# atenpas/gpd

Hardware: AMD Instinct MI355X
Metric: 15-ch grasp candidates scored/sec (imagegen+LeNet) at 1/2/4/8 MI355X (higher is better)
Workload: dtype f64 geometry / u8 images / LeNet f32-equivalent by exact operand splitting: conv1 int8 digit planes of 32-bit fixed-point weights (i32 accumulate, exact), conv2 + ip1 three bf16 pieces per operand (six exact products per term, f32 accumulate), ip2 f32

## Files before the change

### gpd_amd/csrc/images.hip

```cpp
#include <cfloat>
#include <cmath>
#include <cstdio>
#include <cstdlib>
#include <cstring>

#include <mutex>
#include <type_traits>

#include "gpd_internal.h"

namespace gpd {

#define HIP_RET(expr)                                                                       \
  do {                                                                                      \
    hipError_t e_ = (expr);                                                                 \
    if (e_ != hipSuccess) {                                                                 \
      set_error("%s failed: %s (%s:%d)", #expr, hipGetErrorString(e_), __FILE__, __LINE__); \
      return GPD_ERR_HIP;                                                                   \
    }                                                                                       \
  } while (0)

constexpr int IMG_THREADS = 512;
constexpr int SET_THREADS = 1024;
constexpr int IMG_WAVES = IMG_THREADS / 64;
constexpr int PT_CAP = 1024;
constexpr int PT_CAP_BIG = 32768;
constexpr int SH_CAP = 6144;
constexpr int SH_CAP_BIG = 12288;
template <bool WIDE>
struct Vox {
  static constexpr int VD = WIDE ? 64 : 46;
  static constexpr int SD = WIDE ? 128 : 86;
  static constexpr int SR = WIDE ? 64 : 43;
  static constexpr int LB = 18;
  static constexpr int SETWORDS = (SD * SD * SD + 31) / 32;
};

struct ImgConsts {
  double vol_depth, vol_width, vol_height, half_od, dbl_h;
  int C, nproj, per;
  double shadow_length, voxel, voxel_mult, rand_inv;
  int num_shadow;
  uint32_t stride_a, stride_c;
  double len[3];
  double inv_cell[3];
  double thr[3][kImg + 1];
  double inv_len[3];
  int true_div;
  int set_sd, set_sr;
};
__constant__ ImgConsts c_img;

struct ImgParams {
  const float *nn;
  int cap;
  const double *centers;
  const gpd_hand *hands;
  const int32_t *cand_hand;
  const int32_t *meta;
  const uint32_t *set_bits;
  uint8_t *images;
  int32_t *status;
  int num_cand;
  const int32_t *cand_list;
  const int32_t *cand_count;
  int32_t *overflow_list;
  int32_t *overflow_count;
  unsigned long long *dbg;
  int32_t *pts_overflow_list;
  int32_t *pts_overflow_count;
  char *pts_scratch;
  int exit_after;
  char *huge_scratch;
};

struct Box {
  double F[9];
  double sample[3];
  double off[3];
  double lo[3], hi[3];
};

constexpr size_t PTS_SCRATCH_BYTES = (size_t)PT_CAP_BIG * (3 * sizeof(double) + sizeof(float4) + sizeof(uint32_t));
struct PointArrays {
  double t[3][PT_CAP];
  float4 an[PT_CAP];
};
struct NoPointArrays {};
template <bool BIG>
struct __attribute__((aligned(16))) SmemPts {
  typename std::conditional<BIG, NoPointArrays, PointArrays>::type p;
  __attribute__((aligned(16))) uint32_t cells[kPix];
  uint16_t place[BIG ? PT_CAP_BIG : PT_CAP];
  float4 nzv[(BIG ? kPix : PT_CAP) + 1];
  uint16_t nzlist[BIG ? kPix : PT_CAP];
  double thr[3][kImg + 1];
  double recip[128];
  float red_f[4 * IMG_WAVES];
  int red_i[IMG_WAVES];
  int counter;
  int flag;
};
typedef SmemPts<false> Smem;
template <int SHC, bool WIDE>
struct __attribute__((aligned(16))) SmemShadow {
  __attribute__((aligned(16))) float raster0[kPix];
  __attribute__((aligned(16))) uint32_t cells[kPix];
  uint32_t lin[SHC];
  union {
    struct {
      uint16_t rowbase[Vox<WIDE>::VD * Vox<WIDE>::VD];
      uint8_t rowcnt[Vox<WIDE>::VD * Vox<WIDE>::VD];
    } rows;
    uint16_t place[SHC];
  } bp;
  uint16_t nz[kPix];
  uint8_t cz[SHC];
  double thr[3][kImg + 1];
  double recip[128];
  float red_f[4 * IMG_WAVES];
  int red_i[IMG_WAVES];
  int vorg[3];
  int flag;
};

__device__ inline double uniform_f64(double v) {
  const unsigned long long b = (unsigned long long)__double_as_longlong(v);
  const unsigned lo = __builtin_amdgcn_readfirstlane((unsigned)b);
  const unsigned hi = __builtin_amdgcn_readfirstlane((unsigned)(b >> 32));
  return __longlong_as_double((long long)(((unsigned long long)hi << 32) | lo));
}

template <class OP>
__device__ inline float wave_reduce_f32(float v, OP op) {
  auto dpp = [](float x, auto ctrl, auto rmask) {
    return __int_as_float(__builtin_amdgcn_update_dpp(__float_as_int(x), __float_as_int(x), decltype(ctrl)::value, decltype(rmask)::value, 0xf, false));
  };
  using std::integral_constant;
  v = op(v, dpp(v, integral_constant<int, 0xB1>(), integral_constant<int, 0xf>()));
  v = op(v, dpp(v, integral_constant<int, 0x4E>(), integral_constant<int, 0xf>()));
  v = op(v, dpp(v, integral_constant<int, 0x141>(), integral_constant<int, 0xf>()));
  v = op(v, dpp(v, integral_constant<int, 0x140>(), integral_constant<int, 0xf>()));
  v = op(v, dpp(v, integral_constant<int, 0x142>(), integral_constant<int, 0xa>()));
  v = op(v, dpp(v, integral_constant<int, 0x143>(), integral_constant<int, 0xc>()));
  return __int_as_float(__builtin_amdgcn_readlane(__float_as_int(v), 63));
}
__device__ inline float wave_max_f32(float v) { return wave_reduce_f32(v, [](float a, float b) { return fmaxf(a, b); }); }
__device__ inline float wave_min_f32(float v) { return wave_reduce_f32(v, [](float a, float b) { return fminf(a, b); }); }

__device__ inline int wave_incl_scan_i32(int v) {
  v += __builtin_amdgcn_update_dpp(0, v, 0x111, 0xf, 0xf, false);
  v += __builtin_amdgcn_update_dpp(0, v, 0x112, 0xf, 0xf, false);
  v += __builtin_amdgcn_update_dpp(0, v, 0x114, 0xf, 0xf, false);
  v += __builtin_amdgcn_update_dpp(0, v, 0x118, 0xf, 0xf, false);
  v += __builtin_amdgcn_update_dpp(0, v, 0x142, 0xa, 0xf, false);
  v += __builtin_amdgcn_update_dpp(0, v, 0x143, 0xc, 0xf, false);
  return v;
}

__device__ inline void to_hand(const Box &B, double w0, double w1, double w2, double t[3]) {
  const double c0 = w0 - B.sample[0], c1 = w1 - B.sample[1], c2 = w2 - B.sample[2];
  t[0] = B.F[0] * c0 + B.F[3] * c1 + B.F[6] * c2;
  t[1] = B.F[1] * c0 + B.F[4] * c1 + B.F[7] * c2;
  t[2] = B.F[2] * c0 + B.F[5] * c1 + B.F[8] * c2;
}
__device__ inline bool in_box(const Box &B, const double t[3]) {
  return (t[0] > B.lo[0]) && (t[0] < B.hi[0]) && (t[1] > B.lo[1]) && (t[1] < B.hi[1]) && (t[2] > B.lo[2]) && (t[2] < B.hi[2]);
}
template <class SM>
__device__ inline int cell_coord(const SM &S, int axis, double x) {
  int k = (int)(x * c_img.inv_cell[axis]);
  k = k < 0 ? 0 : (k > kImg - 1 ? kImg - 1 : k);
  const double t0 = S.thr[axis][k], t1 = S.thr[axis][k + 1];
  if (k > 0 && x < t0) {
    k--;
    while (k > 0 && x < S.thr[axis][k]) k--;
  } else if (k < kImg - 1 && x >= t1) {
    k++;
    while (k < kImg - 1 && x >= S.thr[axis][k + 1]) k++;
  }
  return k;
}
template <class SM>
__device__ inline uint32_t cells_of(const SM &S, const Box &B, const double t[3]) {
  const int cx = cell_coord(S, 0, t[0] - B.off[0]);
  const int cy = cell_coord(S, 1, t[1] - B.off[1]);
  const int cz = cell_coord(S, 2, t[2] - B.off[2]);
  return (uint32_t)cx | ((uint32_t)cy << 6) | ((uint32_t)cz << 12);
}
__device__ inline int cell_of_key(uint32_t key, int pr) {
  const int cx = key & 63, cy = (key >> 6) & 63, cz = (key >> 12) & 63;
  const int v = pr == 0 ? cx : cz;
  const int h = pr == 2 ? cx : cy;
  return h + v * kImg;
}
__device__ inline int depth_axis(int pr) { return pr == 0 ? 2 : (pr == 1 ? 0 : 1); }

__device__ inline double div_len(double x, int axis) {
  const ImgConsts &K = c_img;
  if (K.true_div) return x / K.len[axis];
  const double y = K.inv_len[axis];
  const double q = x * y;
  const double r = __builtin_fma(-K.len[axis], q, x);
  return __builtin_fma(r, y, q);
}
template <int NTAB>
__device__ inline double recip_count(const double *tab, float fc) {
  const int k = (int)fc;
  return k < NTAB ? tab[k] : 1.0 / (double)fc;
}

__device__ inline uint32_t lcg_step(uint32_t &s) {
  s = 214013u * s + 2531011u;
  return (uint32_t)(((int32_t)s >> 16) & 0x7FFF);
}
__device__ inline uint32_t lcg_jump(uint32_t s, unsigned long long n) {
  uint32_t a = 214013u, c = 2531011u, A = 1u, Cc = 0u;
  while (n) {
    if (n & 1ull) {
      A = a * A;
      Cc = a * Cc + c;
    }
    c = (a + 1u) * c;
    a = a * a;
    n >>= 1;
  }
  return A * s + Cc;
}

template <class SM>
__device__ inline int block_excl_scan(SM &S, int v, int *total) {
  const int lane = threadIdx.x & 63, wave = threadIdx.x >> 6;
  const int incl = wave_incl_scan_i32(v);
  __syncthreads();
  if (lane == 63) S.red_i[wave] = incl;
  __syncthreads();
  int base = 0, tot = 0;
#pragma unroll
  for (int w = 0; w < IMG_WAVES; w++) {
    const int x = S.red_i[w];
    if (w < wave) base += x;
    tot += x;
  }
  *total = tot;
  return base + incl - v;
}

template <class SM>
__device__ int scan_cells(SM &S) {
  const int tid = threadIdx.x;
  constexpr int PER = 8;
  static_assert(kPix % PER == 0 && kPix / PER <= IMG_THREADS, "scan_cells: cells per thread");
  uint4 *c4 = reinterpret_cast<uint4 *>(S.cells);
  if (tid < 32) reinterpret_cast<int *>(S.red_f)[tid] = 0;
  uint4 a = make_uint4(0u, 0u, 0u, 0u), b = a;
  if (tid < kPix / PER) {
    a = c4[2 * tid];
    b = c4[2 * tid + 1];
  }
  const int c[PER] = {(int)(a.x & 0xffffu), (int)(a.y & 0xffffu), (int)(a.z & 0xffffu), (int)(a.w & 0xffffu),
                      (int)(b.x & 0xffffu), (int)(b.y & 0xffffu), (int)(b.z & 0xffffu), (int)(b.w & 0xffffu)};
  int sum = 0;
#pragma unroll
  for (int k = 0; k < PER; k++) sum += c[k];
  int total;
  int run = block_excl_scan(S, sum, &total);
  uint32_t o[PER];
#pragma unroll
  for (int k = 0; k < PER; k++) {
    o[k] = (uint32_t)(run < 0xffff ? run : 0xffff) << 16;
    run += c[k];
  }
  if (tid < kPix / PER) {
    c4[2 * tid] = make_uint4(o[0], o[1], o[2], o[3]);
    c4[2 * tid + 1] = make_uint4(o[4], o[5], o[6], o[7]);
  }
  __syncthreads();
  return total;
}

template <class SM>
__device__ int list_nonempty_cells(SM &S, uint16_t *nz) {
  const int tid = threadIdx.x;
  constexpr int PER = (kPix + IMG_THREADS - 1) / IMG_THREADS;
  int *hist = reinterpret_cast<int *>(S.red_f);
  static_assert(PER == 8, "two 16-byte reads per thread");
  uint4 a = make_uint4(0u, 0u, 0u, 0u), b = a;
  if (tid < kPix / PER) {
    a = reinterpret_cast<const uint4 *>(S.cells)[2 * tid];
    b = reinterpret_cast<const uint4 *>(S.cells)[2 * tid + 1];
  }
  const uint32_t cw[PER] = {a.x, a.y, a.z, a.w, b.x, b.y, b.z, b.w};
  int bucket[PER];
#pragma unroll
  for (int k = 0; k < PER; k++) {
    const int cn = (int)(cw[k] & 0xffffu);
    bucket[k] = cn ? 31 - (cn < 31 ? cn : 31) : -1;
    if (cn) atomicAdd(&hist[bucket[k]], 1);
  }
  __syncthreads();
  if (tid < 64) {
    const int v = tid < 32 ? hist[tid] : 0;
    const int incl = wave_incl_scan_i32(v);
    if (tid < 32) hist[tid] = incl - v;
    if (tid == 31) S.red_i[0] = incl;
  }
  __syncthreads();
#pragma unroll
  for (int k = 0; k < PER; k++)
    if (bucket[k] >= 0) nz[atomicAdd(&hist[bucket[k]], 1)] = (uint16_t)(tid * PER + k);
  __syncthreads();
  return S.red_i[0];
}

template <int NPL, class SM>
__device__ void finalize_planes(SM &S, const float *p012, const float *p3, uint8_t *out) {
  const int tid = threadIdx.x;
  constexpr int GROUPS = NPL * 900;
  constexpr int PER = (GROUPS + IMG_THREADS - 1) / IMG_THREADS;
  float d[PER][4];
  float mn[2] = {FLT_MAX, FLT_MAX}, mx[2] = {-FLT_MAX, -FLT_MAX};
#pragma unroll
  for (int k = 0; k < PER; k++) {
    const int g = tid + k * IMG_THREADS;
    if (g < GROUPS) {
      const int ch = g / 900, rem = g - ch * 900;
      const int r = rem / 15, c0 = (rem - r * 15) * 4;
      const float *pl = (ch < 3) ? p012 + ch * kPix : p3;
      const int rm = r > 0 ? r - 1 : 0, rp = r < kImg - 1 ? r + 1 : kImg - 1;
      const int cl = c0 > 0 ? c0 - 1 : 0, cr = c0 + 4 < kImg ? c0 + 4 : kImg - 1;
      const float4 a = *reinterpret_cast<const float4 *>(pl + rm * kImg + c0);
      const float4 b = *reinterpret_cast<const float4 *>(pl + r * kImg + c0);
      const float4 c = *reinterpret_cast<const float4 *>(pl + rp * kImg + c0);
      const float el = fmaxf(fmaxf(pl[rm * kImg + cl], pl[r * kImg + cl]), pl[rp * kImg + cl]);
      const float er = fmaxf(fmaxf(pl[rm * kImg + cr], pl[r * kImg + cr]), pl[rp * kImg + cr]);
      const float m0 = fmaxf(fmaxf(a.x, b.x), c.x), m1 = fmaxf(fmaxf(a.y, b.y), c.y);
      const float m2 = fmaxf(fmaxf(a.z, b.z), c.z), m3 = fmaxf(fmaxf(a.w, b.w), c.w);
      d[k][0] = fmaxf(fmaxf(el, m0), m1);
      d[k][1] = fmaxf(fmaxf(m0, m1), m2);
      d[k][2] = fmaxf(fmaxf(m1, m2), m3);
      d[k][3] = fmaxf(fmaxf(m2, m3), er);
      const float lo = fminf(fminf(d[k][0], d[k][1]), fminf(d[k][2], d[k][3]));
      const float hi = fmaxf(fmaxf(d[k][0], d[k][1]), fmaxf(d[k][2], d[k][3]));
      if (ch < 3) {
        mn[0] = fminf(mn[0], lo);
        mx[0] = fmaxf(mx[0], hi);
      } else {
        mn[1] = fminf(mn[1], lo);
        mx[1] = fmaxf(mx[1], hi);
      }
    }
  }
#pragma unroll
  for (int q = 0; q < 2; q++) {
    mn[q] = wave_min_f32(mn[q]);
    mx[q] = wave_max_f32(mx[q]);
  }
  __syncthreads();
  if ((tid & 63) == 0) {
    S.red_f[4 * (tid >> 6) + 0] = mn[0];
    S.red_f[4 * (tid >> 6) + 1] = mx[0];
    S.red_f[4 * (tid >> 6) + 2] = mn[1];
    S.red_f[4 * (tid >> 6) + 3] = mx[1];
  }
  __syncthreads();
  float fs[2], fb[2];
#pragma unroll
  for (int q = 0; q < 2; q++) {
    float a = S.red_f[2 * q], b = S.red_f[2 * q + 1];
#pragma unroll
    for (int w = 1; w < IMG_WAVES; w++) {
      a = fminf(a, S.red_f[4 * w + 2 * q]);
      b = fmaxf(b, S.red_f[4 * w + 2 * q + 1]);
    }
    const double smin = (double)a, smax = (double)b;
    const double scale = 1.0 * ((smax - smin) > DBL_EPSILON ? 1.0 / (smax - smin) : 0.0);
    const double shift = 0.0 - smin * scale;
    fs[q] = (float)scale;
    fb[q] = (float)shift;
  }
#pragma unroll
  for (int k = 0; k < PER; k++) {
    const int g = tid + k * IMG_THREADS;
// ... 152 lines not shown
  for (int q = 0; q < 16; q++) k[q] = 16 + q < n ? (uint32_t)p[16 + q] : 0xffffffffu;
  merge_regs<16>(k);
#pragma unroll
  for (int q = 0; q < 16; q++)
    if (16 + q < n) p[16 + q] = (uint16_t)k[q];
}
template <int N>
__device__ inline void sort_regs(uint32_t (&k)[N]) {
#pragma unroll
  for (int size = 2; size <= N; size <<= 1) {
#pragma unroll
    for (int stride = size >> 1; stride > 0; stride >>= 1) {
#pragma unroll
      for (int i = 0; i < N; i++) {
        const int j = i ^ stride;
        if (j > i) {
          const uint32_t lo = min(k[i], k[j]), hi = max(k[i], k[j]);
          const bool up = (i & size) == 0;
          k[i] = up ? lo : hi;
          k[j] = up ? hi : lo;
        }
      }
    }
  }
}
template <int N>
__device__ inline void sort_u16_regs(uint16_t *p, int n) {
  uint32_t k[N];
#pragma unroll
  for (int q = 0; q < N; q++) k[q] = q < n ? (uint32_t)p[q] : 0xffffffffu;
  sort_regs<N>(k);
#pragma unroll
  for (int q = 0; q < N; q++)
    if (q < n) p[q] = (uint16_t)k[q];
}
#define TICK(k)                                                     \
  do {                                                              \
    if (P.dbg && tid == 0) {                                        \
      const unsigned long long now_ = __builtin_readcyclecounter(); \
      atomicAdd(&P.dbg[k], now_ - t_last);                          \
      t_last = now_;                                                \
    }                                                               \
  } while (0)

__device__ inline void load_box(const gpd_hand &H, Box &B) {
  const ImgConsts &K = c_img;
#pragma unroll
  for (int i = 0; i < 9; i++) B.F[i] = uniform_f64(H.frame[i]);
#pragma unroll
  for (int i = 0; i < 3; i++) B.sample[i] = uniform_f64(H.sample[i]);
  const double hb = uniform_f64(H.bottom), hc = uniform_f64(H.center);
  B.off[0] = hb;
  B.off[1] = uniform_f64(hc - K.half_od);
  B.off[2] = uniform_f64(-K.vol_height);
  B.lo[0] = hb;
  B.hi[0] = uniform_f64(hb + K.vol_depth);
  B.lo[1] = B.off[1];
  B.hi[1] = uniform_f64(hc + K.half_od);
  B.lo[2] = uniform_f64(-1.0 * K.vol_height);
  B.hi[2] = uniform_f64(K.vol_height);
}

__device__ __forceinline__ int xcd_candidate(int n) {
  const int per = (n + 7) >> 3;
  const int L = blockIdx.x, slot = L >> 3;
  const int cand = (L & 7) * per + slot;
  return cand < n ? cand : -1;
}

template <int SHC, bool WIDE>
__device__ __forceinline__ void shadow_image_body(const ImgParams &P, SmemShadow<SHC, WIDE> &S, const int cand) {
  constexpr int VDIM = Vox<WIDE>::VD, SD = Vox<WIDE>::SD, SR = Vox<WIDE>::SR, LB = Vox<WIDE>::LB, SETWORDS = Vox<WIDE>::SETWORDS;
  unsigned long long t_last = __builtin_readcyclecounter();
  const ImgConsts &K = c_img;
  const int tid = threadIdx.x;
  const int lane = tid & 63;
  const int set_ord = P.meta[4 * cand + 2];
  const int set_nb = P.meta[4 * cand + 3];
  uint8_t *out = P.images + (size_t)cand * kPix * K.C;
  Box B;
  load_box(P.hands[P.cand_hand[cand]], B);
  for (int i = tid; i < 3 * (kImg + 1); i += IMG_THREADS) (&S.thr[0][0])[i] = (&K.thr[0][0])[i];
  for (int i = tid; i < 128; i += IMG_THREADS) S.recip[i] = i ? 1.0 / (double)i : 0.0;
  if (tid == 0) {
    S.flag = 0;
    double lo[3] = {DBL_MAX, DBL_MAX, DBL_MAX}, hi[3] = {-DBL_MAX, -DBL_MAX, -DBL_MAX};
#pragma unroll
    for (int k = 0; k < 8; k++) {
      const double bx = (k & 1) ? B.hi[0] : B.lo[0];
      const double by = (k & 2) ? B.hi[1] : B.lo[1];
      const double bz = (k & 4) ? B.hi[2] : B.lo[2];
#pragma unroll
      for (int a = 0; a < 3; a++) {
        const double w = B.sample[a] + B.F[3 * a] * bx + B.F[3 * a + 1] * by + B.F[3 * a + 2] * bz;
        lo[a] = fmin(lo[a], w);
        hi[a] = fmax(hi[a], w);
      }
    }
    int bad = 0;
#pragma unroll
    for (int a = 0; a < 3; a++) {
      const int v0 = (int)floor(lo[a] * K.voxel_mult) - 1, v1 = (int)floor(hi[a] * K.voxel_mult) + 1;
      const int o = (int)floor(B.sample[a] * K.voxel_mult) - SR;
      S.vorg[a] = v0;
      if (v1 - v0 >= VDIM || v0 + 1 < o || v1 - 1 >= o + SD) bad = 1;
    }
    S.flag = bad;
  }
  __syncthreads();
  const int x0 = S.vorg[0], y0 = S.vorg[1], z0 = S.vorg[2];
  constexpr int NROWS = VDIM * VDIM, RPT = (NROWS + IMG_THREADS - 1) / IMG_THREADS;
  unsigned long long mask[RPT];
#pragma unroll
  for (int k = 0; k < RPT; k++) mask[k] = 0ull;
  if (set_ord >= 0) {
    const uint32_t *sb = P.set_bits + (size_t)set_ord * SETWORDS;
    const int ox = (int)floor(B.sample[0] * K.voxel_mult) - SR, oy = (int)floor(B.sample[1] * K.voxel_mult) - SR,
              oz = (int)floor(B.sample[2] * K.voxel_mult) - SR;
    const int zlo = z0 - oz;
    double invBz[3];
#pragma unroll
    for (int a = 0; a < 3; a++) {
      const double bz = B.F[6 + a] * K.voxel;
      invBz[a] = uniform_f64(fabs(bz) > 1e-9 ? 1.0 / bz : 0.0);
    }
    const int za = zlo < 0 ? 0 : zlo, zb = (zlo + VDIM < SD) ? zlo + VDIM : SD;
    const int nbits = zb - za;
    double T0[3], Ax[3], Ay[3], Lf[3], Wd[3];
    {
      const double wx = (double)x0 * K.voxel - B.sample[0], wy = (double)y0 * K.voxel - B.sample[1],
                   wz = (double)(za - zlo + z0) * K.voxel - B.sample[2];
#pragma unroll
      for (int a = 0; a < 3; a++) {
        T0[a] = uniform_f64(B.F[a] * wx + B.F[3 + a] * wy + B.F[6 + a] * wz);
        Ax[a] = uniform_f64(B.F[a] * K.voxel);
        Ay[a] = uniform_f64(B.F[3 + a] * K.voxel);
        Lf[a] = invBz[a] > 0.0 ? B.lo[a] : B.hi[a];
        Wd[a] = uniform_f64(fabs((B.hi[a] - B.lo[a]) * invBz[a]));
      }
    }
    unsigned long long fld[RPT];
#pragma unroll
    for (int k = 0; k < RPT; k++) fld[k] = 0ull;
    for (int cb = 0; cb < set_nb; cb++) {
      const uint32_t *sc = sb + (size_t)cb * SETWORDS;
      uint32_t wa[RPT], wb[RPT], wc[RPT];
#pragma unroll
      for (int k = 0; k < RPT; k++) {
        const int row = tid + k * IMG_THREADS;
        const int ix = row / VDIM, iy = row - ix * VDIM;
        const int sx = x0 + ix - ox, sy = y0 + iy - oy;
        const bool ok = row < NROWS && (unsigned)sx < (unsigned)SD && (unsigned)sy < (unsigned)SD && za < zb;
        const int w0 = ok ? ((sx * SD + sy) * SD + za) >> 5 : 0;
        wa[k] = sc[w0];
        wb[k] = sc[w0 + 1 < SETWORDS ? w0 + 1 : SETWORDS - 1];
        wc[k] = sc[w0 + 2 < SETWORDS ? w0 + 2 : SETWORDS - 1];
      }
#pragma unroll
      for (int k = 0; k < RPT; k++) {
        const int row = tid + k * IMG_THREADS;
        const int ix = row / VDIM, iy = row - ix * VDIM;
        const int sx = x0 + ix - ox, sy = y0 + iy - oy;
        const bool ok = row < NROWS && (unsigned)sx < (unsigned)SD && (unsigned)sy < (unsigned)SD && za < zb;
        const int b0 = ok ? (sx * SD + sy) * SD + za : 0;
        const int w0 = b0 >> 5, sh = b0 & 31;
        const unsigned long long lo64 = (unsigned long long)wa[k] | ((unsigned long long)(w0 + 1 < SETWORDS ? wb[k] : 0u) << 32);
        const unsigned long long hi = (w0 + 2 < SETWORDS) ? wc[k] : 0u;
        const unsigned long long f = (lo64 >> sh) | (sh ? (hi << (64 - sh)) : 0ull);
// ... 46 lines not shown
        }
      }
      while (field) {
        const int t = __ffsll((long long)field) - 1;
        field &= field - 1;
        const int iz = za + t - zlo;
        double th[3];
        to_hand(B, (double)(ix + x0) * K.voxel, (double)(iy + y0) * K.voxel, (double)(iz + z0) * K.voxel, th);
        if (in_box(B, th)) mask[k] |= 1ull << iz;
      }
    }
  }
#pragma unroll
  for (int k = 0; k < RPT; k++) {
    const int row = tid + k * IMG_THREADS;
    if (row < NROWS) S.bp.rows.rowcnt[row] = (uint8_t)__popcll(mask[k]);
  }
  __syncthreads();
  TICK(0);
  int cnt = 0;
#pragma unroll
  for (int k = 0; k < RPT; k++) {
    const int row = tid * RPT + k;
    if (row < NROWS) cnt += S.bp.rows.rowcnt[row];
  }
  int n_sh;
  int pos = block_excl_scan(S, cnt, &n_sh);
  if (n_sh > SHC) {
    if (tid == 0) {
      if (P.overflow_list) {
        const int slot = atomicAdd(P.overflow_count, 1);
        P.overflow_list[slot] = cand;
      } else {
        atomicOr(P.status, 4);
      }
    }
    return;
  }
#pragma unroll
  for (int k = 0; k < RPT; k++) {
    const int row = tid * RPT + k;
    if (row < NROWS) {
      S.bp.rows.rowbase[row] = (uint16_t)pos;
      pos += S.bp.rows.rowcnt[row];
    }
  }
  __syncthreads();
#pragma unroll
  for (int k = 0; k < RPT; k++) {
    const int row = tid + k * IMG_THREADS;
    if (row >= NROWS) continue;
    unsigned long long m = mask[k];
    int at = S.bp.rows.rowbase[row];
    const int rx = row / VDIM, ry = row - rx * VDIM;
    const uint32_t rowpos = ((uint32_t)rx << 12) | ((uint32_t)ry << 6);
    while (m) {
      const int iz = __ffsll((long long)m) - 1;
      m &= m - 1;
      S.lin[at++] = rowpos | (uint32_t)iz;
    }
  }
  __syncthreads();
  const int ns = n_sh < SHC ? n_sh : SHC;
  if (P.dbg && tid == 0) {
    atomicMax(&P.dbg[28], (unsigned long long)n_sh);
    atomicAdd(&P.dbg[29], (unsigned long long)n_sh);
  }
  for (int k = tid; k < ns; k += IMG_THREADS) {
    const int lin = (int)S.lin[k];
    const int ix = lin >> 12, iy = (lin >> 6) & 63, iz = lin & 63;
    double th[3];
    to_hand(B, (double)(ix + x0) * K.voxel, (double)(iy + y0) * K.voxel, (double)(iz + z0) * K.voxel, th);
    const uint32_t c3 = cells_of(S, B, th);
    S.lin[k] = (uint32_t)lin | ((c3 & 0xfffu) << LB);
    S.cz[k] = (uint8_t)(c3 >> 12);
  }
  __syncthreads();
  TICK(1);
  auto cell_of_entry = [&](int k, int pr) {
    const uint32_t v = S.lin[k];
    return cell_of_key(((v >> LB) & 0xfffu) | ((uint32_t)S.cz[k] << 12), pr);
  };
  for (int pr = 0; pr < 3; pr++) {
    for (int c = tid; c < kPix / 4; c += IMG_THREADS) reinterpret_cast<uint4 *>(S.cells)[c] = make_uint4(0u, 0u, 0u, 0u);
    __syncthreads();
    for (int k = tid; k < ns; k += IMG_THREADS) atomicAdd(&S.cells[cell_of_entry(k, pr)], 1u);
    __syncthreads();
    scan_cells(S);
    for (int k = tid; k < ns; k += IMG_THREADS) {
      const uint32_t old = atomicAdd(&S.cells[cell_of_entry(k, pr)], 1u);
      S.bp.place[(old >> 16) + (old & 0xffffu)] = (uint16_t)k;
    }
    __syncthreads();
    TICK(2);
    const int da = depth_axis(pr);
    const double Fd0 = da == 0 ? B.F[0] : (da == 1 ? B.F[1] : B.F[2]);
    const double Fd1 = da == 0 ? B.F[3] : (da == 1 ? B.F[4] : B.F[5]);
    const double Fd2 = da == 0 ? B.F[6] : (da == 1 ? B.F[7] : B.F[8]);
    const double offd = da == 0 ? B.off[0] : (da == 1 ? B.off[1] : B.off[2]);
    float lmax = -FLT_MAX;
    int lany = 0;
    const int n_nz = list_nonempty_cells(S, S.nz);
    for (int c = tid; c < kPix / 4; c += IMG_THREADS) reinterpret_cast<float4 *>(S.raster0)[c] = make_float4(0.f, 0.f, 0.f, 0.f);
    __syncthreads();
    TICK(9);
    for (int qn = tid; qn < n_nz; qn += IMG_THREADS) {
      const int c = S.nz[qn];
      const uint32_t w = S.cells[c];
      const int cn = (int)(w & 0xffffu), start = (int)(w >> 16);
      float v = 0.f, fc = 0.f;
      auto visit = [&](int k) {
        const int lin = (int)(S.lin[k] & ((1u << LB) - 1u));
        const int ix = lin >> 12, iy = (lin >> 6) & 63, iz = lin & 63;
        const double c0 = (double)(ix + x0) * K.voxel - B.sample[0], c1 = (double)(iy + y0) * K.voxel - B.sample[1],
                     c2 = (double)(iz + z0) * K.voxel - B.sample[2];
        const double td = Fd0 * c0 + Fd1 * c1 + Fd2 * c2;
        const double d = div_len(td - offd, da);
        fc = (float)((double)fc + 1.0);
        v = (float)((double)v + (d - (double)v) * recip_count<128>(S.recip, fc));
      };
      sort_u16(&S.bp.place[start], cn);
      for (int e = 0; e < cn; e++) visit((int)S.bp.place[start + e]);
      lmax = fmaxf(lmax, v);
      lany = 1;
      S.raster0[c] = v;
    }
    __syncthreads();
    TICK(10);
    lmax = wave_max_f32(lmax);
    lany = __ballot(lany != 0) != 0ull;
    if (lane == 0) {
      S.red_f[tid >> 6] = lmax;
      S.red_i[tid >> 6] = lany;
    }
    __syncthreads();
    float gmax = -FLT_MAX;
    int gany = 0;
#pragma unroll
    for (int w = 0; w < IMG_WAVES; w++) {
      gmax = fmaxf(gmax, S.red_f[w]);
      gany |= S.red_i[w];
    }
    const double mxd = gany ? (double)gmax : 0.0;
    const float mxf = (float)mxd;
    for (int c = tid; c < kPix / 4; c += IMG_THREADS) {
      const uint4 w = reinterpret_cast<const uint4 *>(S.cells)[c];
      float4 r = reinterpret_cast<float4 *>(S.raster0)[c];
      r.x = ((w.x & 0xffffu) ? mxf : 0.0f) - r.x;
      r.y = ((w.y & 0xffffu) ? mxf : 0.0f) - r.y;
      r.z = ((w.z & 0xffffu) ? mxf : 0.0f) - r.z;
      r.w = ((w.w & 0xffffu) ? mxf : 0.0f) - r.w;
      reinterpret_cast<float4 *>(S.raster0)[c] = r;
    }
    __syncthreads();
    TICK(3);
    finalize_planes<1>(S, &S.raster0[0], nullptr, out + (size_t)(pr * K.per + 4) * kPix);
    TICK(4);
  }
  if (tid == 0 && S.flag) atomicOr(P.status, S.flag);
}

constexpr int LGRID = 256;

template <int SHC, bool WIDE>
__global__ __launch_bounds__(IMG_THREADS, SHC <= SH_CAP ? 4 : 2) void shadow_image_kernel(ImgParams P) {
  __shared__ SmemShadow<SHC, WIDE> S;
  if constexpr (SHC > SH_CAP) {
    const int count = *P.cand_count;
    for (int q = blockIdx.x; q < count; q += gridDim.x) {
      __syncthreads();
      shadow_image_body<SHC, WIDE>(P, S, P.cand_list[q]);
    }
  } else {
    const int cand = xcd_candidate(P.num_cand);
    if (cand < 0) return;
    shadow_image_body<SHC, WIDE>(P, S, cand);
  }
}

constexpr int HUGE_CAP = 65535;
constexpr int HUGE_WIN = 256;
constexpr size_t HUGE_SCRATCH_BYTES = (size_t)HUGE_WIN * HUGE_WIN * sizeof(int32_t) + (size_t)(HUGE_CAP + 1) * (2 * sizeof(uint32_t) + sizeof(uint16_t)) + 64;
struct __attribute__((aligned(16))) SmemAny {
  __attribute__((aligned(16))) float raster0[kPix];
  __attribute__((aligned(16))) uint32_t cells[kPix];
  uint16_t nz[kPix];
  double thr[3][kImg + 1];
  double recip[128];
  float red_f[4 * IMG_WAVES];
  int red_i[IMG_WAVES];
  int vorg[3], wdim[3];
  int flag;
};

__device__ void shadow_image_any_body(const ImgParams &P, SmemAny &S, const int cand, char *scratch) {
  const ImgConsts &K = c_img;
  const int SD = K.set_sd, SR = K.set_sr;
  const size_t SETWORDS = (size_t)(((long long)SD * SD * SD + 31) / 32);
  const int tid = threadIdx.x;
  const int lane = tid & 63;
  const int set_ord = P.meta[4 * cand + 2];
  const int set_nb = P.meta[4 * cand + 3];
  uint8_t *out = P.images + (size_t)cand * kPix * K.C;
  int32_t *rowtab = reinterpret_cast<int32_t *>(scratch);
  uint32_t *lin = reinterpret_cast<uint32_t *>(rowtab + HUGE_WIN * HUGE_WIN);
  uint32_t *ckey = lin + (HUGE_CAP + 1);
  uint16_t *place = reinterpret_cast<uint16_t *>(ckey + (HUGE_CAP + 1));
  Box B;
  load_box(P.hands[P.cand_hand[cand]], B);
  for (int i = tid; i < 3 * (kImg + 1); i += IMG_THREADS) (&S.thr[0][0])[i] = (&K.thr[0][0])[i];
  for (int i = tid; i < 128; i += IMG_THREADS) S.recip[i] = i ? 1.0 / (double)i : 0.0;
  if (tid == 0) {
    double lo[3] = {DBL_MAX, DBL_MAX, DBL_MAX}, hi[3] = {-DBL_MAX, -DBL_MAX, -DBL_MAX};
    for (int k = 0; k < 8; k++) {
      const double bx = (k & 1) ? B.hi[0] : B.lo[0];
      const double by = (k & 2) ? B.hi[1] : B.lo[1];
      const double bz = (k & 4) ? B.hi[2] : B.lo[2];
      for (int a = 0; a < 3; a++) {
        const double w = B.sample[a] + B.F[3 * a] * bx + B.F[3 * a + 1] * by + B.F[3 * a + 2] * bz;
        lo[a] = fmin(lo[a], w);
        hi[a] = fmax(hi[a], w);
      }
    }
    int bad = 0;
    for (int a = 0; a < 3; a++) {
      const int v0 = (int)floor(lo[a] * K.voxel_mult) - 1, v1 = (int)floor(hi[a] * K.voxel_mult) + 1;
      const int o = (int)floor(B.sample[a] * K.voxel_mult) - SR;
      S.vorg[a] = v0;
      S.wdim[a] = v1 - v0 + 1;
      if (v1 - v0 + 1 > HUGE_WIN || v0 + 1 < o || v1 - 1 >= o + SD) bad = 1;
    }
    S.flag = bad;
  }
  __syncthreads();
  if (S.flag) {
    if (tid == 0) atomicOr(P.status, 1);
    return;
  }
  const int x0 = S.vorg[0], y0 = S.vorg[1], z0 = S.vorg[2];
  const int wx = S.wdim[0], wy = S.wdim[1], wz = S.wdim[2];
  const int nrows = wx * wy;
  const int ox = (int)floor(B.sample[0] * K.voxel_mult) - SR, oy = (int)floor(B.sample[1] * K.voxel_mult) - SR,
            oz = (int)floor(B.sample[2] * K.voxel_mult) - SR;
  auto walk_row = [&](int row, auto emit) {
    const int ix = row / wy, iy = row - ix * wy;
    const int sx = x0 + ix - ox, sy = y0 + iy - oy;
    if (set_ord < 0 || (unsigned)sx >= (unsigned)SD || (unsigned)sy >= (unsigned)SD) return;
    const int zlo = z0 - oz;
    const int za = zlo < 0 ? 0 : zlo, zb = zlo + wz < SD ? zlo + wz : SD;
    if (za >= zb) return;
    const long long rowbit = ((long long)sx * SD + sy) * SD;
    for (long long w = (rowbit + za) >> 5; w <= (rowbit + zb - 1) >> 5; w++) {
      uint32_t bits = ~0u;
      for (int cb = 0; cb < set_nb; cb++) bits &= P.set_bits[((size_t)set_ord + cb) * SETWORDS + (size_t)w];
      const long long first = w << 5;
      if (first < rowbit + za) bits &= ~0u << (int)(rowbit + za - first);
      if (first + 32 > rowbit + zb) bits &= ~0u >> (int)(first + 32 - (rowbit + zb));
      while (bits) {
        const int t = __ffs((int)bits) - 1;
        bits &= bits - 1;
        const int iz = (int)(first + t - rowbit) - zlo;
        double th[3];
        to_hand(B, (double)(ix + x0) * K.voxel, (double)(iy + y0) * K.voxel, (double)(iz + z0) * K.voxel, th);
        if (in_box(B, th)) emit(iz);
      }
    }
  };
  for (int row = tid; row < nrows; row += IMG_THREADS) {
    int cnt = 0;
    walk_row(row, [&](int) { cnt++; });
    rowtab[row] = cnt;
  }
  __threadfence_block();
  __syncthreads();
  const int per = (nrows + IMG_THREADS - 1) / IMG_THREADS;
  int cnt = 0;
  for (int k = 0; k < per; k++) {
    const int row = tid * per + k;
    if (row < nrows) cnt += rowtab[row];
  }
  int n_sh;
  int pos = block_excl_scan(S, cnt, &n_sh);
  if (n_sh > HUGE_CAP) {
    if (tid == 0) atomicOr(P.status, 4);
    return;
  }
  for (int k = 0; k < per; k++) {
    const int row = tid * per + k;
    if (row < nrows) {
      const int c = rowtab[row];
      rowtab[row] = pos;
      pos += c;
    }
  }
  __threadfence_block();
  __syncthreads();
  for (int row = tid; row < nrows; row += IMG_THREADS) {
    int at = rowtab[row];
    const int ix = row / wy, iy = row - ix * wy;
    walk_row(row, [&](int iz) {
      double th[3];
      to_hand(B, (double)(ix + x0) * K.voxel, (double)(iy + y0) * K.voxel, (double)(iz + z0) * K.voxel, th);
      lin[at] = (uint32_t)ix | ((uint32_t)iy << 8) | ((uint32_t)iz << 16);
      ckey[at] = cells_of(S, B, th);
      at++;
    });
  }
  __threadfence_block();
  __syncthreads();
  const int ns = n_sh;
  for (int pr = 0; pr < 3; pr++) {
    for (int c = tid; c < kPix; c += IMG_THREADS) S.cells[c] = 0u;
    __syncthreads();
    for (int k = tid; k < ns; k += IMG_THREADS) atomicAdd(&S.cells[cell_of_key(ckey[k], pr)], 1u);
    __syncthreads();
    scan_cells(S);
    for (int k = tid; k < ns; k += IMG_THREADS) {
      const uint32_t old = atomicAdd(&S.cells[cell_of_key(ckey[k], pr)], 1u);
      place[(old >> 16) + (old & 0xffffu)] = (uint16_t)k;
    }
    __threadfence_block();
    __syncthreads();
    const int da = depth_axis(pr);
    const double Fd0 = da == 0 ? B.F[0] : (da == 1 ? B.F[1] : B.F[2]);
    const double Fd1 = da == 0 ? B.F[3] : (da == 1 ? B.F[4] : B.F[5]);
    const double Fd2 = da == 0 ? B.F[6] : (da == 1 ? B.F[7] : B.F[8]);
    const double offd = da == 0 ? B.off[0] : (da == 1 ? B.off[1] : B.off[2]);
    float lmax = -FLT_MAX;
    int lany = 0;
    const int n_nz = list_nonempty_cells(S, S.nz);
    for (int c = tid; c < kPix; c += IMG_THREADS) S.raster0[c] = 0.f;
    __syncthreads();
    for (int qn = tid; qn < n_nz; qn += IMG_THREADS) {
      const int c = S.nz[qn];
      const uint32_t w = S.cells[c];
      const int cn = (int)(w & 0xffffu), start = (int)(w >> 16);
      float v = 0.f, fc = 0.f;
      sort_u16(&place[start], cn);
      for (int e = 0; e < cn; e++) {
        const uint32_t lp = lin[place[start + e]];
        const int ix = lp & 255, iy = (lp >> 8) & 255, iz = lp >> 16;
        const double c0 = (double)(ix + x0) * K.voxel - B.sample[0], c1 = (double)(iy + y0) * K.voxel - B.sample[1],
                     c2 = (double)(iz + z0) * K.voxel - B.sample[2];
        const double td = Fd0 * c0 + Fd1 * c1 + Fd2 * c2;
        const double d = div_len(td - offd, da);
        fc = (float)((double)fc + 1.0);
        v = (float)((double)v + (d - (double)v) * recip_count<128>(S.recip, fc));
      }
      lmax = fmaxf(lmax, v);
      lany = 1;
      S.raster0[c] = v;
    }
    __syncthreads();
    lmax = wave_max_f32(lmax);
    lany = __ballot(lany != 0) != 0ull;
    if (lane == 0) {
      S.red_f[tid >> 6] = lmax;
      S.red_i[tid >> 6] = lany;
    }
    __syncthreads();
    float gmax = -FLT_MAX;
    int gany = 0;
    for (int w = 0; w < IMG_WAVES; w++) {
      gmax = fmaxf(gmax, S.red_f[w]);
      gany |= S.red_i[w];
    }
    const double mxd = gany ? (double)gmax : 0.0;
    const float mxf = (float)mxd;
    __syncthreads();
    for (int c = tid; c < kPix; c += IMG_THREADS) S.raster0[c] = ((S.cells[c] & 0xffffu) ? mxf : 0.0f) - S.raster0[c];
    __syncthreads();
    finalize_planes<1>(S, &S.raster0[0], nullptr, out + (size_t)(pr * K.per + 4) * kPix);
  }
}

__global__ __launch_bounds__(IMG_THREADS) void shadow_image_any_kernel(ImgParams P) {
  __shared__ SmemAny S;
  char *scratch = P.huge_scratch + (size_t)blockIdx.x * HUGE_SCRATCH_BYTES;
  const int count = P.cand_list ? *P.cand_count : P.num_cand;
  for (int q = blockIdx.x; q < count; q += gridDim.x) {
    __syncthreads();
    shadow_image_any_body(P, S, P.cand_list ? P.cand_list[q] : q, scratch);
  }
}

template <bool BIG>
__device__ __forceinline__ void grasp_image_body(const ImgParams &P, SmemPts<BIG> &S, const int cand) {
  constexpr int CAP = BIG ? PT_CAP_BIG : PT_CAP;
  unsigned long long t_last = __builtin_readcyclecounter();
  const ImgConsts &K = c_img;
  const int tid = threadIdx.x;
  const int lane = tid & 63;
  const int slot_s = P.meta[4 * cand + 0];
  const int N = P.meta[4 * cand + 1];
  const float *nn = P.nn + (size_t)slot_s * 6 * P.cap;
  uint8_t *out = P.images + (size_t)cand * kPix * K.C;
// ... 48 lines not shown
#pragma unroll
      for (int q = 0; q < 4; q++) {
        const int r = r0 + q;
        const int i = b0 + r * IMG_THREADS + tid;
        double t[3];
        to_hand(B, (double)px[q], (double)py[q], (double)pz[q], t);
        const bool in = i < N && in_box(B, t);
        const unsigned long long ballot = __ballot(in);
        if (lane == 0) cnt[r * IMG_WAVES + wave] = __popcll(ballot);
        inmask |= (unsigned)in << r;
      }
    }
    __syncthreads();
    int run = n_before;
    for (int r = 0; r < nr; r++) {
      int base = run;
#pragma unroll
      for (int w = 0; w < IMG_WAVES; w++) {
        const int c = cnt[r * IMG_WAVES + w];
        if (w < wave) base += c;
        run += c;
      }
      const bool in = (inmask >> r) & 1u;
      const unsigned long long ballot = __ballot(in);
      if (in) {
        const int e = base + __popcll(ballot & ((1ull << lane) - 1ull));
        if (e < CAP) {
          if constexpr (BIG) gidx[e] = (uint32_t)(b0 + r * IMG_THREADS + tid);
          else S.place[e] = (uint16_t)(b0 + r * IMG_THREADS + tid);
        }
      }
    }
    n_before = run;
    __syncthreads();
  }
  const int n_box_all = n_before;
  if (n_box_all > CAP || (!BIG && N > 65536)) {
    if (tid == 0) {
      if (!BIG && P.pts_overflow_list)
        P.pts_overflow_list[atomicAdd(P.pts_overflow_count, 1)] = cand;
      else
        atomicOr(P.status, 2);
    }
    return;
  }
  for (int e0 = 0; e0 < n_box_all; e0 += 2 * IMG_THREADS) {
    float v[2][6];
#pragma unroll
    for (int q = 0; q < 2; q++) {
      const int e = e0 + q * IMG_THREADS + tid;
      const int i = e < n_box_all ? IDX(e) : 0;
#pragma unroll
      for (int a = 0; a < 6; a++) v[q][a] = nn[a * P.cap + i];
    }
#pragma unroll
    for (int q = 0; q < 2; q++) {
      const int e = e0 + q * IMG_THREADS + tid;
      if (e < n_box_all) {
        double t[3];
        to_hand(B, (double)v[q][0], (double)v[q][1], (double)v[q][2], t);
        const double n0 = (double)v[q][3], n1 = (double)v[q][4], n2 = (double)v[q][5];
        T(0, e) = t[0];
        T(1, e) = t[1];
        T(2, e) = t[2];
        AN(e) = make_float4((float)fabs(B.F[0] * n0 + B.F[3] * n1 + B.F[6] * n2),
                            (float)fabs(B.F[1] * n0 + B.F[4] * n1 + B.F[7] * n2),
                            (float)fabs(B.F[2] * n0 + B.F[5] * n1 + B.F[8] * n2), __uint_as_float(cells_of(S, B, t)));
      }
    }
  }
  if constexpr (BIG) {
    __threadfence_block();
    __syncthreads();
  }
  const int nb = n_box_all;
  if (P.dbg && tid == 0) {
    atomicMax(&P.dbg[30], (unsigned long long)n_box_all);
    atomicAdd(&P.dbg[31], (unsigned long long)n_box_all);
  }
  TICK(5);
  for (int c = tid; c < kPix / 4; c += IMG_THREADS) reinterpret_cast<uint4 *>(S.cells)[c] = make_uint4(0u, 0u, 0u, 0u);
  __syncthreads();
  for (int pr = 0; pr < K.nproj; pr++) {
    for (int e = tid; e < nb; e += IMG_THREADS) atomicAdd(&S.cells[cell_of_key(__float_as_uint(AN(e).w), pr)], 1u);
    __syncthreads();
    scan_cells(S);
    for (int e = tid; e < nb; e += IMG_THREADS) {
      const uint32_t key = __float_as_uint(AN(e).w);
      const uint32_t old = atomicAdd(&S.cells[cell_of_key(key, pr)], 1u);
      S.place[(old >> 16) + (old & 0xffffu)] = (uint16_t)e;
    }
    __syncthreads();
    TICK(6);
    const int da = depth_axis(pr);
    const double offd = da == 0 ? B.off[0] : (da == 1 ? B.off[1] : B.off[2]);
    uint16_t *nz = S.nzlist;
    const int n_nz = list_nonempty_cells(S, nz);
    TICK(11);
    for (int qn = tid; qn < n_nz; qn += IMG_THREADS) {
      const int c = nz[qn];
      const uint32_t w = S.cells[c];
      const int cn = (int)(w & 0xffffu), start = (int)(w >> 16);
      float v0 = 0.f, v1 = 0.f, v2 = 0.f;
      float avg = 0.f, fc = 0.f;
      auto visit = [&](int e) {
        const float4 an = AN(e);
        const float a0 = an.x, a1 = an.y, a2 = an.z;
        if (v0 == 0.f && v1 == 0.f && v2 == 0.f) {
          v0 = a0;
          v1 = a1;
          v2 = a2;
        } else {
          const float sq = sqrtf(v0 * v0 + v1 * v1 + v2 * v2);
          const double inv = 1.0 / (double)sq;
          const float d0 = a0 - v0, d1 = a1 - v1, d2 = a2 - v2;
          v0 = v0 + (float)((double)d0 * inv);
          v1 = v1 + (float)((double)d1 * inv);
          v2 = v2 + (float)((double)d2 * inv);
        }
        const double d = div_len(T(da, e) - offd, da);
        fc = (float)((double)fc + 1.0);
        avg = (float)((double)avg + (d - (double)avg) * recip_count<128>(S.recip, fc));
      };
      sort_u16_lean(&S.place[start], cn);
      for (int q = 0; q < cn; q++) visit((int)S.place[start + q]);
      S.nzv[qn + 1] = make_float4(v0, v1, v2, (float)(1.0 - (double)avg));
      S.cells[c] = 0x80000000u | (uint32_t)(qn + 1);
    }
    TICK(13);
    __syncthreads();
    TICK(7);
    const bool with_normals = K.C != 1, with_depth = K.C == 1 || K.C >= 12;
    uint16_t *alist = S.place;
    if (tid == 0) S.counter = 0;
    __syncthreads();
    bool live[GPT];
    auto window = [&](int g, uint32_t(&ix)[3][6]) {
      const int r = g / 15, c0 = (g - r * 15) * 4;
      const int rows[3] = {r > 0 ? r - 1 : 0, r, r < kImg - 1 ? r + 1 : kImg - 1};
      const int cl = c0 > 0 ? c0 - 1 : 0, cr = c0 + 4 < kImg ? c0 + 4 : kImg - 1;
      uint32_t any = 0;
#pragma unroll
      for (int q = 0; q < 3; q++) {
        const uint4 m = *reinterpret_cast<const uint4 *>(&S.cells[rows[q] * kImg + c0]);
        ix[q][0] = S.cells[rows[q] * kImg + cl];
        ix[q][1] = m.x;
        ix[q][2] = m.y;
        ix[q][3] = m.z;
        ix[q][4] = m.w;
        ix[q][5] = S.cells[rows[q] * kImg + cr];
#pragma unroll
        for (int e = 0; e < 6; e++) any |= ix[q][e];
      }
      return (any >> 31) != 0u;
    };
    TICK(12);
#pragma unroll
    for (int k = 0; k < GPT; k++) {
      const int g = tid + k * IMG_THREADS;
      uint32_t ix[3][6];
      live[k] = g < 900 && window(g, ix);
      const unsigned long long ballot = __ballot(live[k]);
      if (ballot) {
        int base = 0;
        if (lane == 0) base = atomicAdd(&S.counter, __popcll(ballot));
        base = __builtin_amdgcn_readfirstlane(base);
// ... 668 lines not shown
```

Measured before the change: 2.176 million.

## Restructure shadow projection: sparse dilation over live groups, fused normalization, merged histogram

```diff
diff --git a/gpd_amd/csrc/images.hip b/gpd_amd/csrc/images.hip
--- a/gpd_amd/csrc/images.hip
+++ b/gpd_amd/csrc/images.hip
@@ -104,8 +104,9 @@
 typedef SmemPts<false> Smem;
 template <int SHC, bool WIDE>
 struct __attribute__((aligned(16))) SmemShadow {
-  __attribute__((aligned(16))) float raster0[kPix];
   __attribute__((aligned(16))) uint32_t cells[kPix];
+  float val[kPix + 1];
+  int counter;
   uint32_t lin[SHC];
   union {
     struct {
@@ -247,12 +248,18 @@
 }
 
 template <class SM>
+__device__ inline void clear_length_buckets(SM &S) {
+  if (threadIdx.x < 32) reinterpret_cast<int *>(S.red_f)[threadIdx.x] = 0;
+}
+__device__ inline int length_bucket(int cn) { return 31 - (cn < 31 ? cn : 31); }
+
+template <class SM>
 __device__ int scan_cells(SM &S) {
   const int tid = threadIdx.x;
   constexpr int PER = 8;
   static_assert(kPix % PER == 0 && kPix / PER <= IMG_THREADS, "scan_cells: cells per thread");
   uint4 *c4 = reinterpret_cast<uint4 *>(S.cells);
-  if (tid < 32) reinterpret_cast<int *>(S.red_f)[tid] = 0;
+  int *hist = reinterpret_cast<int *>(S.red_f);
   uint4 a = make_uint4(0u, 0u, 0u, 0u), b = a;
   if (tid < kPix / PER) {
     a = c4[2 * tid];
@@ -262,7 +269,10 @@
                       (int)(b.x & 0xffffu), (int)(b.y & 0xffffu), (int)(b.z & 0xffffu), (int)(b.w & 0xffffu)};
   int sum = 0;
 #pragma unroll
-  for (int k = 0; k < PER; k++) sum += c[k];
+  for (int k = 0; k < PER; k++) {
+    sum += c[k];
+    if (c[k]) atomicAdd(&hist[length_bucket(c[k])], 1);
+  }
   int total;
   int run = block_excl_scan(S, sum, &total);
   uint32_t o[PER];
@@ -295,10 +305,8 @@
 #pragma unroll
   for (int k = 0; k < PER; k++) {
     const int cn = (int)(cw[k] & 0xffffu);
-    bucket[k] = cn ? 31 - (cn < 31 ? cn : 31) : -1;
-    if (cn) atomicAdd(&hist[bucket[k]], 1);
-  }
-  __syncthreads();
+    bucket[k] = cn ? length_bucket(cn) : -1;
+  }
   if (tid < 64) {
     const int v = tid < 32 ? hist[tid] : 0;
     const int incl = wave_incl_scan_i32(v);
@@ -617,8 +625,10 @@
   load_box(P.hands[P.cand_hand[cand]], B);
   for (int i = tid; i < 3 * (kImg + 1); i += IMG_THREADS) (&S.thr[0][0])[i] = (&K.thr[0][0])[i];
   for (int i = tid; i < 128; i += IMG_THREADS) S.recip[i] = i ? 1.0 / (double)i : 0.0;
+  for (int c = tid; c < kPix / 4; c += IMG_THREADS) reinterpret_cast<uint4 *>(S.cells)[c] = make_uint4(0u, 0u, 0u, 0u);
   if (tid == 0) {
     S.flag = 0;
+    S.val[0] = 0.f;
     double lo[3] = {DBL_MAX, DBL_MAX, DBL_MAX}, hi[3] = {-DBL_MAX, -DBL_MAX, -DBL_MAX};
 #pragma unroll
     for (int k = 0; k < 8; k++) {
@@ -831,8 +841,8 @@
     return cell_of_key(((v >> LB) & 0xfffu) | ((uint32_t)S.cz[k] << 12), pr);
   };
   for (int pr = 0; pr < 3; pr++) {
-    for (int c = tid; c < kPix / 4; c += IMG_THREADS) reinterpret_cast<uint4 *>(S.cells)[c] = make_uint4(0u, 0u, 0u, 0u);
-    __syncthreads();
+    clear_length_buckets(S);
+    if (tid == 0) S.counter = 0;
     for (int k = tid; k < ns; k += IMG_THREADS) atomicAdd(&S.cells[cell_of_entry(k, pr)], 1u);
     __syncthreads();
     scan_cells(S);
@@ -848,10 +858,7 @@
     const double Fd2 = da == 0 ? B.F[6] : (da == 1 ? B.F[7] : B.F[8]);
     const double offd = da == 0 ? B.off[0] : (da == 1 ? B.off[1] : B.off[2]);
     float lmax = -FLT_MAX;
-    int lany = 0;
     const int n_nz = list_nonempty_cells(S, S.nz);
-    for (int c = tid; c < kPix / 4; c += IMG_THREADS) reinterpret_cast<float4 *>(S.raster0)[c] = make_float4(0.f, 0.f, 0.f, 0.f);
-    __syncthreads();
     TICK(9);
     for (int qn = tid; qn < n_nz; qn += IMG_THREADS) {
       const int c = S.nz[qn];
@@ -871,39 +878,134 @@
       sort_u16(&S.bp.place[start], cn);
       for (int e = 0; e < cn; e++) visit((int)S.bp.place[start + e]);
       lmax = fmaxf(lmax, v);
-      lany = 1;
-      S.raster0[c] = v;
+      S.val[qn + 1] = v;
+      S.cells[c] = 0x80000000u | (uint32_t)(qn + 1);
     }
     __syncthreads();
     TICK(10);
+    int ft = tid;
+    asm volatile("" : "+v"(ft));
     lmax = wave_max_f32(lmax);
-    lany = __ballot(lany != 0) != 0ull;
+    if (lane == 0) S.red_f[2 * IMG_WAVES + (ft >> 6)] = lmax;
+    uint16_t *alist = S.bp.place;
+    auto window = [&](int g, uint32_t(&ix)[3][6]) {
+      const int r = g / 15, c0 = (g - r * 15) * 4;
+      const int rows[3] = {r > 0 ? r - 1 : 0, r, r < kImg - 1 ? r + 1 : kImg - 1};
+      const int cl = c0 > 0 ? c0 - 1 : 0, cr = c0 + 4 < kImg ? c0 + 4 : kImg - 1;
+      uint32_t any = 0;
+#pragma unroll
+      for (int q = 0; q < 3; q++) {
+        const uint4 m = *reinterpret_cast<const uint4 *>(&S.cells[rows[q] * kImg + c0]);
+        ix[q][0] = S.cells[rows[q] * kImg + cl];
+        ix[q][1] = m.x;
+        ix[q][2] = m.y;
+        ix[q][3] = m.z;
+        ix[q][4] = m.w;
+        ix[q][5] = S.cells[rows[q] * kImg + cr];
+#pragma unroll
+        for (int e = 0; e < 6; e++) any |= ix[q][e];
+      }
+      return (any >> 31) != 0u;
+    };
+#pragma unroll
+    for (int k = 0; k < GPT; k++) {
+      const int g = ft + k * IMG_THREADS;
+      uint32_t ix[3][6];
+      const bool live = g < 900 && window(g, ix);
+      const unsigned long long ballot = __ballot(live);
+      if (ballot) {
+        int base = 0;
+        if (lane == 0) base = atomicAdd(&S.counter, __popcll(ballot));
+        base = __builtin_amdgcn_readfirstlane(base);
+        if (live) alist[base + __popcll(ballot & ((1ull << lane) - 1ull))] = (uint16_t)g;
+      }
+    }
+    __syncthreads();
+    TICK(3);
+    const int n_live = S.counter;
+    float gmax = -FLT_MAX;
+#pragma unroll
+    for (int w = 0; w < IMG_WAVES; w++) gmax = fmaxf(gmax, S.red_f[2 * IMG_WAVES + w]);
+    const double mxd = n_nz > 0 ? (double)gmax : 0.0;
+    const float mxf = (float)mxd;
+    auto value = [&](uint32_t w) {
+      const uint32_t slot = (w >> 31) ? (w & 0xffffu) : 0u;
+      const float x = S.val[slot];
+      return slot ? mxf - x : 0.0f;
+    };
+    float d[GPT][4];
+    float mn = FLT_MAX, mx = -FLT_MAX;
+    if (n_live < 900) mn = mx = 0.f;
+#pragma unroll
+    for (int k = 0; k < GPT; k++) {
+      const int a = ft + k * IMG_THREADS;
+      if (a < n_live) {
+        uint32_t ix[3][6];
+        window((int)alist[a], ix);
+        float col[6];
+#pragma unroll
+        for (int e = 0; e < 6; e++) col[e] = fmaxf(fmaxf(value(ix[0][e]), value(ix[1][e])), value(ix[2][e]));
+#pragma unroll
+        for (int j = 0; j < 4; j++) d[k][j] = fmaxf(fmaxf(col[j], col[j + 1]), col[j + 2]);
+        mn = fminf(mn, fminf(fminf(d[k][0], d[k][1]), fminf(d[k][2], d[k][3])));
+        mx = fmaxf(mx, fmaxf(fmaxf(d[k][0], d[k][1]), fmaxf(d[k][2], d[k][3])));
+      }
+    }
+    if (64 * (ft >> 6) < n_live) {
+      mn = wave_min_f32(mn);
+      mx = wave_max_f32(mx);
+    }
     if (lane == 0) {
-      S.red_f[tid >> 6] = lmax;
-      S.red_i[tid >> 6] = lany;
-    }
-    __syncthreads();
-    float gmax = -FLT_MAX;
-    int gany = 0;
-#pragma unroll
-    for (int w = 0; w < IMG_WAVES; w++) {
-      gmax = fmaxf(gmax, S.red_f[w]);
-      gany |= S.red_i[w];
-    }
-    const double mxd = gany ? (double)gmax : 0.0;
-    const float mxf = (float)mxd;
-    for (int c = tid; c < kPix / 4; c += IMG_THREADS) {
-      const uint4 w = reinterpret_cast<const uint4 *>(S.cells)[c];
-      float4 r = reinterpret_cast<float4 *>(S.raster0)[c];
-      r.x = ((w.x & 0xffffu) ? mxf : 0.0f) - r.x;
-      r.y = ((w.y & 0xffffu) ? mxf : 0.0f) - r.y;
-      r.z = ((w.z & 0xffffu) ? mxf : 0.0f) - r.z;
-      r.w = ((w.w & 0xffffu) ? mxf : 0.0f) - r.w;
-      reinterpret_cast<float4 *>(S.raster0)[c] = r;
-    }
-    __syncthreads();
-    TICK(3);
-    finalize_planes<1>(S, &S.raster0[0], nullptr, out + (size_t)(pr * K.per + 4) * kPix);
+      S.red_f[2 * (ft >> 6)] = mn;
+      S.red_f[2 * (ft >> 6) + 1] = mx;
+    }
+    __syncthreads();
+    auto to_byte = [](float x, float s, float b) {
+      const float v = x * s + b;
+      const float u = v * 255.0f + 0.0f;
+      float t = rintf(u);
+      t = t < 0.f ? 0.f : (t > 255.f ? 255.f : t);
+      return (uint32_t)(int)t;
+    };
+    float fs, fb;
+    {
+      float a = S.red_f[0], b = S.red_f[1];
+#pragma unroll
+      for (int w = 1; w < IMG_WAVES; w++) {
+        a = fminf(a, S.red_f[2 * w]);
+        b = fmaxf(b, S.red_f[2 * w + 1]);
+      }
+      const double smin = (double)a, smax = (double)b;
+      const double scale = 1.0 * ((smax - smin) > DBL_EPSILON ? 1.0 / (smax - smin) : 0.0);
+      const double shift = 0.0 - smin * scale;
+      fs = (float)scale;
+      fb = (float)shift;
+    }
+    const uint32_t bg = to_byte(0.f, fs, fb) * 0x01010101u;
+    uint32_t *stage = S.cells;
+    uint4 *stage4 = reinterpret_cast<uint4 *>(S.cells);
+    for (int c = ft; c < 225; c += IMG_THREADS) stage4[c] = make_uint4(bg, bg, bg, bg);
+    __syncthreads();
+#pragma unroll
+    for (int k = 0; k < GPT; k++) {
+      const int a = ft + k * IMG_THREADS;
+      if (a < n_live) {
+        const int g = (int)alist[a];
+        const int r = g / 15, cg = g - r * 15;
+        uint32_t packed = 0;
+#pragma unroll
+        for (int j = 0; j < 4; j++) packed |= to_byte(d[k][j], fs, fb) << (8 * j);
+        stage[(kImg - 1 - r) * 15 + cg] = packed;
+      }
+    }
+    __syncthreads();
+    uint8_t *plane = out + (size_t)(pr * K.per + 4) * kPix;
+    for (int a = ft; a < kPix / 4; a += IMG_THREADS) {
+      const uint4 v = stage4[a];
+      stage4[a] = make_uint4(0u, 0u, 0u, 0u);
+      if (a < 225) *reinterpret_cast<uint4 *>(plane + 16 * a) = v;
+    }
+    __syncthreads();
     TICK(4);
   }
   if (tid == 0 && S.flag) atomicOr(P.status, S.flag);
@@ -930,6 +1032,7 @@
 constexpr int HUGE_CAP = 65535;
 constexpr int HUGE_WIN = 256;
 constexpr size_t HUGE_SCRATCH_BYTES = (size_t)HUGE_WIN * HUGE_WIN * sizeof(int32_t) + (size_t)(HUGE_CAP + 1) * (2 * sizeof(uint32_t) + sizeof(uint16_t)) + 64;
+static_assert(sizeof(SmemShadow<SH_CAP, false>) <= 81680, "shadow_image_kernel<SH_CAP>: two workgroups per CU");
 struct __attribute__((aligned(16))) SmemAny {
   __attribute__((aligned(16))) float raster0[kPix];
   __attribute__((aligned(16))) uint32_t cells[kPix];
@@ -1061,6 +1164,7 @@
   for (int pr = 0; pr < 3; pr++) {
     for (int c = tid; c < kPix; c += IMG_THREADS) S.cells[c] = 0u;
     __syncthreads();
+    clear_length_buckets(S);
     for (int k = tid; k < ns; k += IMG_THREADS) atomicAdd(&S.cells[cell_of_key(ckey[k], pr)], 1u);
     __syncthreads();
     scan_cells(S);
@@ -1275,6 +1379,7 @@
   for (int c = tid; c < kPix / 4; c += IMG_THREADS) reinterpret_cast<uint4 *>(S.cells)[c] = make_uint4(0u, 0u, 0u, 0u);
   __syncthreads();
   for (int pr = 0; pr < K.nproj; pr++) {
+    clear_length_buckets(S);
     for (int e = tid; e < nb; e += IMG_THREADS) atomicAdd(&S.cells[cell_of_key(__float_as_uint(AN(e).w), pr)], 1u);
     __syncthreads();
     scan_cells(S);
```

New measurement: 2.142 million. 0.984x the previous value.
